# OliBus801/TARL-simulator

Hardware: AMD Instinct MI355X
Metric: ppo_env_steps_per_sec (higher is better)
Workload: dtype f32; 1 GPU; mpnn+ppo train, 10000-edge torus dual graph, 16384 agents, T=256 (BASELINE config 4); envs_per_gpu=32768, parallelism=dp1, rollout_kernels=frames

## Files before the change

### tarl-simulator_amd/csrc/critic.hip

```cpp
#include "tarl_common.h"

#define CR_H 64
#define CR_BM 128
#define CR_BK 32
#define CR_THREADS 256

typedef float f32x16 __attribute__((ext_vector_type(16)));

struct CriticParams {
  const float* w1;
  const float* b1;
  const float* w2;
  const float* b2;
  const float* w3;
  const float* b3;
};

__device__ __forceinline__ int mfma_row(int reg, int lane) { return (reg & 3) + 8 * (reg >> 2) + 4 * (lane >> 5); }

template <typename XT>
__global__ __launch_bounds__(CR_THREADS) void k_critic_fwd(const XT* __restrict__ counts, int64_t ldc, int64_t rps,
                                                           int64_t M, int64_t N,
                                                           const float* __restrict__ time_rows,
                                                           int64_t rows_per_time, CriticParams P,
                                                           float* __restrict__ value, float* __restrict__ h1_out,
                                                           float* __restrict__ h2_out) {
  __shared__ float lds[CR_H * (CR_BM + 1) + CR_H * (CR_H + 1)];
  float* Xs = lds;
  float* Ws = lds + CR_BK * (CR_BM + 1);
  const int tid = threadIdx.x, lane = tid & 63, wave = tid >> 6;
  const int64_t row0 = (int64_t)blockIdx.x * CR_BM;
  const int64_t ldw = N + 1;

  f32x16 acc0 = {0}, acc1 = {0};
  for (int64_t k0 = 0; k0 < N; k0 += CR_BK) {
    if (rps == 0) {
#pragma unroll
      for (int it = 0; it < (CR_BM * CR_BK) / CR_THREADS; ++it) {
        const int idx = it * CR_THREADS + tid;
        const int r = idx >> 5, k = idx & 31;
        const int64_t gr = row0 + r, gk = k0 + k;
        Xs[k * (CR_BM + 1) + r] = (gr < M && gk < N) ? (float)counts[gr * ldc + gk] : 0.0f;
      }
    } else {
      const int64_t slab_base = (row0 / rps) * (N * rps) + (row0 % rps);
#pragma unroll
      for (int it = 0; it < (CR_BM * CR_BK) / CR_THREADS; ++it) {
        const int idx = it * CR_THREADS + tid;
        const int r = idx & (CR_BM - 1), k = idx >> 7;
        const int64_t gr = row0 + r, gk = k0 + k;
        Xs[k * (CR_BM + 1) + r] = (gr < M && gk < N) ? (float)counts[slab_base + gk * rps + r] : 0.0f;
      }
    }
#pragma unroll
    for (int it = 0; it < (CR_H * CR_BK) / CR_THREADS; ++it) {
      const int idx = it * CR_THREADS + tid;
      const int j = idx >> 5, k = idx & 31;
      const int64_t gk = k0 + k;
      Ws[k * (CR_H + 1) + j] = (gk < N) ? P.w1[(int64_t)j * ldw + gk] : 0.0f;
    }
    __syncthreads();
#pragma unroll
    for (int kk = 0; kk < CR_BK; kk += 2) {
      const int k = kk + (lane >> 5);
      const float a = Xs[k * (CR_BM + 1) + wave * 32 + (lane & 31)];
      const float b0 = Ws[k * (CR_H + 1) + (lane & 31)];
      const float b1 = Ws[k * (CR_H + 1) + 32 + (lane & 31)];
      acc0 = __builtin_amdgcn_mfma_f32_32x32x2f32(a, b0, acc0, 0, 0, 0);
      acc1 = __builtin_amdgcn_mfma_f32_32x32x2f32(a, b1, acc1, 0, 0, 0);
    }
    __syncthreads();
  }

  float* Hs = lds;
  float* W2s = lds + CR_H * (CR_BM + 1);
  {
    const int j0 = lane & 31;
    const float wt0 = P.w1[(int64_t)j0 * ldw + N], wt1 = P.w1[(int64_t)(j0 + 32) * ldw + N];
    const float bb0 = P.b1[j0], bb1 = P.b1[j0 + 32];
#pragma unroll
    for (int r = 0; r < 16; ++r) {
      const int lr = wave * 32 + mfma_row(r, lane);
      const int64_t gr = row0 + lr;
      const float tm = (gr < M) ? time_rows[gr / rows_per_time] : 0.0f;
      float v0 = acc0[r] + tm * wt0 + bb0;
      float v1 = acc1[r] + tm * wt1 + bb1;
      v0 = v0 > 0.0f ? v0 : 0.0f;
      v1 = v1 > 0.0f ? v1 : 0.0f;
      Hs[j0 * (CR_BM + 1) + lr] = v0;
      Hs[(j0 + 32) * (CR_BM + 1) + lr] = v1;
      if (h1_out && gr < M) {
        h1_out[gr * CR_H + j0] = v0;
        h1_out[gr * CR_H + j0 + 32] = v1;
      }
    }
  }
#pragma unroll
  for (int it = 0; it < (CR_H * CR_H) / CR_THREADS; ++it) {
    const int idx = it * CR_THREADS + tid;
    const int j = idx >> 6, k = idx & 63;
    W2s[k * (CR_H + 1) + j] = P.w2[j * CR_H + k];
  }
  __syncthreads();
  f32x16 c0 = {0}, c1 = {0};
#pragma unroll
  for (int kk = 0; kk < CR_H; kk += 2) {
    const int k = kk + (lane >> 5);
    const float a = Hs[k * (CR_BM + 1) + wave * 32 + (lane & 31)];
    const float b0 = W2s[k * (CR_H + 1) + (lane & 31)];
    const float b1 = W2s[k * (CR_H + 1) + 32 + (lane & 31)];
    c0 = __builtin_amdgcn_mfma_f32_32x32x2f32(a, b0, c0, 0, 0, 0);
    c1 = __builtin_amdgcn_mfma_f32_32x32x2f32(a, b1, c1, 0, 0, 0);
  }
  __syncthreads();
  {
    const int j0 = lane & 31;
    const float bb0 = P.b2[j0], bb1 = P.b2[j0 + 32];
#pragma unroll
    for (int r = 0; r < 16; ++r) {
      const int lr = wave * 32 + mfma_row(r, lane);
      const int64_t gr = row0 + lr;
      float v0 = c0[r] + bb0, v1 = c1[r] + bb1;
      v0 = v0 > 0.0f ? v0 : 0.0f;
      v1 = v1 > 0.0f ? v1 : 0.0f;
      Hs[j0 * (CR_BM + 1) + lr] = v0;
      Hs[(j0 + 32) * (CR_BM + 1) + lr] = v1;
      if (h2_out && gr < M) {
        h2_out[gr * CR_H + j0] = v0;
        h2_out[gr * CR_H + j0 + 32] = v1;
      }
    }
  }
  __syncthreads();
  if (tid < CR_BM) {
    const int64_t gr = row0 + tid;
    if (gr < M) {
      float s = 0.0f;
#pragma unroll 8
      for (int j = 0; j < CR_H; ++j) s += Hs[j * (CR_BM + 1) + tid] * P.w3[j];
      value[gr] = s + P.b3[0];
    }
  }
}

#define CRS_LDX (CR_BM + 4)
__device__ __forceinline__ float4 load_x4(const float* p) { return *reinterpret_cast<const float4*>(p); }
__device__ __forceinline__ float4 load_x4(const uint8_t* p) {
  const uint32_t w = *reinterpret_cast<const uint32_t*>(p);
  return make_float4((float)(w & 255u), (float)((w >> 8) & 255u), (float)((w >> 16) & 255u), (float)(w >> 24));
}
template <typename XT>
__global__ __launch_bounds__(CR_THREADS) void k_critic_fwd_slab(const XT* __restrict__ counts, int64_t rps, int64_t M,
                                                                int64_t N, const float* __restrict__ time_rows,
                                                                int64_t rows_per_time, CriticParams P,
                                                                float* __restrict__ value) {
  __shared__ __attribute__((aligned(16))) float lds[2 * (CR_BK * CRS_LDX + CR_BK * (CR_H + 1))];
  const int XS = CR_BK * CRS_LDX, BUF = XS + CR_BK * (CR_H + 1);
  const int tid = threadIdx.x, lane = tid & 63, wave = tid >> 6;
  const int64_t row0 = (int64_t)blockIdx.x * CR_BM;
  const int64_t ldw = N + 1;
  const XT* xbase = counts + (row0 / rps) * (N * rps) + (row0 % rps);

  float4 xr[4];
  float wr[8];
  auto fetch = [&](int64_t k0) {
#pragma unroll
    for (int it = 0; it < 4; ++it) {
      const int idx = it * CR_THREADS + tid;
      const int r4 = (idx & 31) * 4, k = idx >> 5;
      const int64_t gk = k0 + k;
      xr[it] = (gk < N) ? load_x4(xbase + gk * rps + r4) : make_float4(0.f, 0.f, 0.f, 0.f);
    }
#pragma unroll
    for (int it = 0; it < 8; ++it) {
      const int idx = it * CR_THREADS + tid;
      const int j = idx >> 5, k = idx & 31;
      const int64_t gk = k0 + k;
      wr[it] = (gk < N) ? P.w1[(int64_t)j * ldw + gk] : 0.0f;
    }
  };
  auto stash = [&](int buf) {
    float* Xs = lds + buf * BUF;
    float* Ws = Xs + XS;
#pragma unroll
    for (int it = 0; it < 4; ++it) {
      const int idx = it * CR_THREADS + tid;
      const int r4 = (idx & 31) * 4, k = idx >> 5;
      *reinterpret_cast<float4*>(Xs + k * CRS_LDX + r4) = xr[it];
    }
#pragma unroll
    for (int it = 0; it < 8; ++it) {
      const int idx = it * CR_THREADS + tid;
      const int j = idx >> 5, k = idx & 31;
      Ws[k * (CR_H + 1) + j] = wr[it];
    }
  };

  f32x16 acc0 = {0}, acc1 = {0};
  fetch(0);
  stash(0);
  __syncthreads();
  int buf = 0;
  for (int64_t k0 = 0; k0 < N; k0 += CR_BK) {
    const bool more = k0 + CR_BK < N;
    if (more) fetch(k0 + CR_BK);
    const float* Xs = lds + buf * BUF;
    const float* Ws = Xs + XS;
#pragma unroll
    for (int kk = 0; kk < CR_BK; kk += 2) {
      const int k = kk + (lane >> 5);
      const float a = Xs[k * CRS_LDX + wave * 32 + (lane & 31)];
      const float b0 = Ws[k * (CR_H + 1) + (lane & 31)];
      const float b1 = Ws[k * (CR_H + 1) + 32 + (lane & 31)];
      acc0 = __builtin_amdgcn_mfma_f32_32x32x2f32(a, b0, acc0, 0, 0, 0);
      acc1 = __builtin_amdgcn_mfma_f32_32x32x2f32(a, b1, acc1, 0, 0, 0);
    }
    if (more) stash(buf ^ 1);
    __syncthreads();
    buf ^= 1;
  }

  float* Hs = lds;
  float* W2s = lds + CR_H * (CR_BM + 1);
  {
    const int j0 = lane & 31;
    const float wt0 = P.w1[(int64_t)j0 * ldw + N], wt1 = P.w1[(int64_t)(j0 + 32) * ldw + N];
    const float bb0 = P.b1[j0], bb1 = P.b1[j0 + 32];
#pragma unroll
    for (int r = 0; r < 16; ++r) {
      const int lr = wave * 32 + mfma_row(r, lane);
      const int64_t gr = row0 + lr;
      const float tm = (gr < M) ? time_rows[gr / rows_per_time] : 0.0f;
      float v0 = acc0[r] + tm * wt0 + bb0;
      float v1 = acc1[r] + tm * wt1 + bb1;
      v0 = v0 > 0.0f ? v0 : 0.0f;
      v1 = v1 > 0.0f ? v1 : 0.0f;
      Hs[j0 * (CR_BM + 1) + lr] = v0;
      Hs[(j0 + 32) * (CR_BM + 1) + lr] = v1;
    }
  }
#pragma unroll
  for (int it = 0; it < (CR_H * CR_H) / CR_THREADS; ++it) {
    const int idx = it * CR_THREADS + tid;
    const int j = idx >> 6, k = idx & 63;
    W2s[k * (CR_H + 1) + j] = P.w2[j * CR_H + k];
  }
  __syncthreads();
  f32x16 c0 = {0}, c1 = {0};
#pragma unroll
  for (int kk = 0; kk < CR_H; kk += 2) {
    const int k = kk + (lane >> 5);
    const float a = Hs[k * (CR_BM + 1) + wave * 32 + (lane & 31)];
    const float b0 = W2s[k * (CR_H + 1) + (lane & 31)];
    const float b1 = W2s[k * (CR_H + 1) + 32 + (lane & 31)];
    c0 = __builtin_amdgcn_mfma_f32_32x32x2f32(a, b0, c0, 0, 0, 0);
    c1 = __builtin_amdgcn_mfma_f32_32x32x2f32(a, b1, c1, 0, 0, 0);
  }
  __syncthreads();
  {
    const int j0 = lane & 31;
    const float bb0 = P.b2[j0], bb1 = P.b2[j0 + 32];
#pragma unroll
    for (int r = 0; r < 16; ++r) {
      const int lr = wave * 32 + mfma_row(r, lane);
      float v0 = c0[r] + bb0, v1 = c1[r] + bb1;
      v0 = v0 > 0.0f ? v0 : 0.0f;
      v1 = v1 > 0.0f ? v1 : 0.0f;
      Hs[j0 * (CR_BM + 1) + lr] = v0;
      Hs[(j0 + 32) * (CR_BM + 1) + lr] = v1;
    }
  }
  __syncthreads();
  if (tid < CR_BM) {
    const int64_t gr = row0 + tid;
    if (gr < M) {
      float s = 0.0f;
#pragma unroll 8
      for (int j = 0; j < CR_H; ++j) s += Hs[j * (CR_BM + 1) + tid] * P.w3[j];
      value[gr] = s + P.b3[0];
    }
  }
}

typedef __bf16 cbf16x8 __attribute__((ext_vector_type(8)));
#define CB_XLD 36
#define CB_WLD 40

__device__ __forceinline__ uint16_t cr_bf16_rne(float f) {
  uint32_t u = __float_as_uint(f);
  u += 0x7fffu + ((u >> 16) & 1u);
  return (uint16_t)(u >> 16);
}

__global__ __launch_bounds__(CR_THREADS) void k_split_w1(const float* __restrict__ w1, int64_t N, int64_t Kpad,
                                                         uint16_t* __restrict__ w3) {
  const int64_t idx = (int64_t)blockIdx.x * CR_THREADS + threadIdx.x;
  if (idx >= CR_H * Kpad) return;
  const int64_t j = idx / Kpad, k = idx - j * Kpad;
  const float w = k < N ? w1[j * (N + 1) + k] : 0.0f;
  const uint16_t hi = cr_bf16_rne(w);
  const float r1 = w - __uint_as_float((uint32_t)hi << 16);
  const uint16_t mid = cr_bf16_rne(r1);
  const float r2 = r1 - __uint_as_float((uint32_t)mid << 16);
  const uint16_t lo = cr_bf16_rne(r2);
  w3[idx] = hi;
  w3[CR_H * Kpad + idx] = mid;
  w3[2 * CR_H * Kpad + idx] = lo;
}

template <int CT>
__global__ __launch_bounds__(CR_THREADS) void k_critic_fwd_slab_u8x3(const uint8_t* __restrict__ counts, int64_t rps,
                                                                     int64_t M, int64_t N, int64_t Kpad,
                                                                     const float* __restrict__ time_rows,
                                                                     int64_t rows_per_time,
                                                                     const uint16_t* __restrict__ w3, CriticParams P,
                                                                     float* __restrict__ value) {
  constexpr int XB = CT * CR_BM * CB_XLD, WB = 3 * CR_H * CB_WLD * 2, BUF = XB + WB;
  constexpr int EPI = (CR_H * (CR_BM + 1) + CR_H * (CR_H + 1)) * 4;
  __shared__ __attribute__((aligned(16))) uint8_t lds_raw[2 * BUF > EPI ? 2 * BUF : EPI];
  static_assert(CR_BK == 32 && CR_BM == 128 && CR_THREADS == 256 && (CR_BM * CB_XLD) % 16 == 0, "X staging plan");
  const int tid = threadIdx.x, lane = tid & 63, wave = tid >> 6;
  const int64_t row0 = (int64_t)blockIdx.x * (CR_BM * CT);
  const int64_t ldw = N + 1;
  const uint8_t* xbase = counts + (row0 / rps) * (N * rps) + (row0 % rps);
  const int64_t WP = CR_H * Kpad;

  struct XStage {
    uint32_t xr[CT][4];
  };
  typedef uint32_t cu32x4 __attribute__((ext_vector_type(4)));
  struct WStage {
    cu32x4 p0, p1, p2;
  };
  const int64_t NIT = (N + CR_BK - 1) / CR_BK;
  const uint8_t* xthread = xbase + (int64_t)(4 * (tid >> 5)) * rps + 4 * (tid & 31);
  auto fetch_x = [&](XStage& st, int64_t it) __attribute__((always_inline)) {
    const int64_t k0 = (it < NIT ? it : NIT - 1) * CR_BK;
    if (k0 + CR_BK <= N) {
      const uint8_t* xk = xthread + k0 * rps;
#pragma unroll
      for (int i = 0; i < 4; ++i) {
#pragma unroll
        for (int c = 0; c < CT; ++c) st.xr[c][i] = *reinterpret_cast<const uint32_t*>(xk + CR_BM * c);
        xk += rps;
      }
    } else {
      const int kg = tid >> 5, eg = tid & 31;
#pragma unroll
      for (int i = 0; i < 4; ++i) {
        const int64_t k = k0 + 4 * kg + i;
        const uint8_t* xk = xbase + (k < N ? k : N - 1) * rps + 4 * eg;
#pragma unroll
        for (int c = 0; c < CT; ++c) st.xr[c][i] = *reinterpret_cast<const uint32_t*>(xk + CR_BM * c);
      }
    }
  };
  auto fetch_w = [&](WStage& st, int64_t it) __attribute__((always_inline)) {
    const int64_t k0 = (it < NIT ? it : NIT - 1) * CR_BK;
    const int j = tid >> 2, q = tid & 3;
    const uint16_t* wp = w3 + (int64_t)j * Kpad + k0 + 8 * q;
    st.p0 = *reinterpret_cast<const cu32x4*>(wp);
    st.p1 = *reinterpret_cast<const cu32x4*>(wp + WP);
    st.p2 = *reinterpret_cast<const cu32x4*>(wp + 2 * WP);
  };
  auto stash = [&](const XStage& sx, const WStage& sw, int buf) __attribute__((always_inline)) {
    uint8_t* Xs = lds_raw + buf * BUF;
    uint16_t* Wb = reinterpret_cast<uint16_t*>(Xs + XB);
    const int kg = tid >> 5, eg = tid & 31;
#pragma unroll
    for (int c = 0; c < CT; ++c) {
      const uint32_t r0 = sx.xr[c][0], r1 = sx.xr[c][1], r2 = sx.xr[c][2], r3 = sx.xr[c][3];
      const uint32_t a_lo = __builtin_amdgcn_perm(r1, r0, 0x05010400u), a_hi = __builtin_amdgcn_perm(r1, r0, 0x07030602u);
      const uint32_t b_lo = __builtin_amdgcn_perm(r3, r2, 0x05010400u), b_hi = __builtin_amdgcn_perm(r3, r2, 0x07030602u);
      const uint32_t v[4] = {__builtin_amdgcn_perm(b_lo, a_lo, 0x05040100u), __builtin_amdgcn_perm(b_lo, a_lo, 0x07060302u),
                             __builtin_amdgcn_perm(b_hi, a_hi, 0x05040100u), __builtin_amdgcn_perm(b_hi, a_hi, 0x07060302u)};
#pragma unroll
      for (int e = 0; e < 4; ++e) *reinterpret_cast<uint32_t*>(Xs + (CR_BM * c + 4 * eg + e) * CB_XLD + 4 * kg) = v[e];
    }
    const int j = tid >> 2, q = tid & 3;
    *reinterpret_cast<cu32x4*>(Wb + (0 * CR_H + j) * CB_WLD + 8 * q) = sw.p0;
    *reinterpret_cast<cu32x4*>(Wb + (1 * CR_H + j) * CB_WLD + 8 * q) = sw.p1;
    *reinterpret_cast<cu32x4*>(Wb + (2 * CR_H + j) * CB_WLD + 8 * q) = sw.p2;
  };

  f32x16 acc0[CT], acc1[CT];
#pragma unroll
  for (int c = 0; c < CT; ++c) {
    acc0[c] = (f32x16){0};
    acc1[c] = (f32x16){0};
  }
  const int r32 = lane & 31, h8 = (lane >> 5) * 8;
  auto multiply = [&](int buf) __attribute__((always_inline)) {
    const uint8_t* Xs = lds_raw + buf * BUF;
    const uint16_t* Wb = reinterpret_cast<const uint16_t*>(Xs + XB);
#pragma unroll
    for (int s = 0; s < CR_BK / 16; ++s) {
      cbf16x8 bx[CT];
#pragma unroll
      for (int c = 0; c < CT; ++c) {
        const uint32_t* xw = reinterpret_cast<const uint32_t*>(Xs + (CR_BM * c + wave * 32 + r32) * CB_XLD + 16 * s + h8);
        const uint32_t x0 = xw[0], x1 = xw[1];
        uint32_t bw[4];
#pragma unroll
        for (int j = 0; j < 4; ++j) {
          const uint32_t xs = j < 2 ? x0 : x1;
          const float c0 = (float)((xs >> (16 * (j & 1))) & 0xFFu), c1 = (float)((xs >> (16 * (j & 1) + 8)) & 0xFFu);
          bw[j] = __builtin_amdgcn_perm(__float_as_uint(c1), __float_as_uint(c0), 0x07060302u);
        }
        bx[c] = __builtin_bit_cast(cbf16x8, bw);
      }
#pragma unroll
      for (int pc = 0; pc < 3; ++pc) {
        const cbf16x8 a0 = *reinterpret_cast<const cbf16x8*>(Wb + (pc * CR_H + r32) * CB_WLD + 16 * s + h8);
        const cbf16x8 a1 = *reinterpret_cast<const cbf16x8*>(Wb + (pc * CR_H + 32 + r32) * CB_WLD + 16 * s + h8);
#pragma unroll
        for (int c = 0; c < CT; ++c) {
          acc0[c] = __builtin_amdgcn_mfma_f32_32x32x16_bf16(a0, bx[c], acc0[c], 0, 0, 0);
          acc1[c] = __builtin_amdgcn_mfma_f32_32x32x16_bf16(a1, bx[c], acc1[c], 0, 0, 0);
        }
      }
    }
  };
  XStage x0, x1, x2, x3;
  WStage w0, w1;
  fetch_w(w0, 0);
  fetch_x(x0, 0);
  fetch_w(w1, 1);
  fetch_x(x1, 1);
  fetch_x(x2, 2);
  fetch_x(x3, 3);
  stash(x0, w0, 0);
  __syncthreads();
#define CR_STEP(T_, XA_, XB_, WA_, WB_, BUF_)                                           \
  {                                                                                     \
    fetch_w(WA_, (T_) + 2);                                                             \
    fetch_x(XA_, (T_) + 4);                                                             \
    if ((T_) < NIT) multiply(BUF_);           \
    stash(XB_, WB_, (BUF_) ^ 1);                                                        \
    __syncthreads();                                                                    \
  }
  for (int64_t it = 0; it < NIT; it += 4) {
    CR_STEP(it, x0, x1, w0, w1, 0);
    CR_STEP(it + 1, x1, x2, w1, w0, 1);
    CR_STEP(it + 2, x2, x3, w0, w1, 0);
    CR_STEP(it + 3, x3, x0, w1, w0, 1);
  }
#undef CR_STEP

  float* Hs = reinterpret_cast<float*>(lds_raw);
  float* W2s = Hs + CR_H * (CR_BM + 1);
#pragma unroll
  for (int it = 0; it < (CR_H * CR_H) / CR_THREADS; ++it) {
    const int idx = it * CR_THREADS + tid;
    const int j = idx >> 6, k = idx & 63;
    W2s[k * (CR_H + 1) + j] = P.w2[j * CR_H + k];
  }
#pragma unroll
  for (int c = 0; c < CT; ++c) {
    const int64_t rowc = row0 + CR_BM * c;
    {
      const int lr = wave * 32 + r32;
      const int64_t gr = rowc + lr;
      const float tm = (gr < M) ? time_rows[gr / rows_per_time] : 0.0f;
#pragma unroll
      for (int r = 0; r < 16; ++r) {
        const int j = mfma_row(r, lane);
        float v0 = acc0[c][r] + tm * P.w1[(int64_t)j * ldw + N] + P.b1[j];
        float v1 = acc1[c][r] + tm * P.w1[(int64_t)(j + 32) * ldw + N] + P.b1[j + 32];
        Hs[j * (CR_BM + 1) + lr] = v0 > 0.0f ? v0 : 0.0f;
        Hs[(j + 32) * (CR_BM + 1) + lr] = v1 > 0.0f ? v1 : 0.0f;
      }
    }
    __syncthreads();
    f32x16 c0 = {0}, c1 = {0};
#pragma unroll
    for (int kk = 0; kk < CR_H; kk += 2) {
      const int k = kk + (lane >> 5);
      const float a = Hs[k * (CR_BM + 1) + wave * 32 + (lane & 31)];
      const float b0 = W2s[k * (CR_H + 1) + (lane & 31)];
      const float b1 = W2s[k * (CR_H + 1) + 32 + (lane & 31)];
      c0 = __builtin_amdgcn_mfma_f32_32x32x2f32(a, b0, c0, 0, 0, 0);
      c1 = __builtin_amdgcn_mfma_f32_32x32x2f32(a, b1, c1, 0, 0, 0);
    }
    __syncthreads();
    {
      const int j0 = lane & 31;
      const float bb0 = P.b2[j0], bb1 = P.b2[j0 + 32];
#pragma unroll
      for (int r = 0; r < 16; ++r) {
        const int lr = wave * 32 + mfma_row(r, lane);
        float v0 = c0[r] + bb0, v1 = c1[r] + bb1;
        v0 = v0 > 0.0f ? v0 : 0.0f;
        v1 = v1 > 0.0f ? v1 : 0.0f;
        Hs[j0 * (CR_BM + 1) + lr] = v0;
        Hs[(j0 + 32) * (CR_BM + 1) + lr] = v1;
      }
    }
    __syncthreads();
    if (tid < CR_BM) {
      const int64_t gr = rowc + tid;
      if (gr < M) {
        float sacc = 0.0f;
#pragma unroll 8
        for (int j = 0; j < CR_H; ++j) sacc += Hs[j * (CR_BM + 1) + tid] * P.w3[j];
        value[gr] = sacc + P.b3[0];
      }
    }
    __syncthreads();
  }
}

__global__ __launch_bounds__(CR_H) void k_critic_bwd_rows(int64_t M, const float* __restrict__ dv,
                                                          const float* __restrict__ h1, const float* __restrict__ h2,
                                                          CriticParams P, float* __restrict__ dh1,
                                                          float* __restrict__ dh2) {
  __shared__ float s_dh2[CR_H];
  const int64_t m = blockIdx.x;
  const int j = threadIdx.x;
  const float g = dv[m];
  const float d2 = (h2[m * CR_H + j] > 0.0f) ? g * P.w3[j] : 0.0f;
  s_dh2[j] = d2;
  dh2[m * CR_H + j] = d2;
  __syncthreads();
  float s = 0.0f;
  for (int i = 0; i < CR_H; ++i) s += s_dh2[i] * P.w2[i * CR_H + j];
  dh1[m * CR_H + j] = (h1[m * CR_H + j] > 0.0f) ? s : 0.0f;
}

__global__ __launch_bounds__(CR_THREADS) void k_critic_bwd_small(int64_t M, const float* __restrict__ dv,
                                                                 const float* __restrict__ h1,
                                                                 const float* __restrict__ h2,
                                                                 const float* __restrict__ dh1,
                                                                 const float* __restrict__ dh2,
                                                                 const float* __restrict__ time_rows,
                                                                 int64_t rows_per_time, int64_t N,
                                                                 float* __restrict__ gw1, float* __restrict__ gb1,
                                                                 float* __restrict__ gw2, float* __restrict__ gb2,
                                                                 float* __restrict__ gw3, float* __restrict__ gb3) {
  const int idx = blockIdx.x * CR_THREADS + threadIdx.x;
  if (idx < CR_H * CR_H) {
    const int j = idx >> 6, k = idx & 63;
    float s = 0.0f;
    for (int64_t m = 0; m < M; ++m) s += dh2[m * CR_H + j] * h1[m * CR_H + k];
    gw2[idx] += s;
  }
  if (idx < CR_H) {
    float sb2 = 0.0f, sb1 = 0.0f, sw3 = 0.0f, swt = 0.0f;
    for (int64_t m = 0; m < M; ++m) {
      sb2 += dh2[m * CR_H + idx];
      sb1 += dh1[m * CR_H + idx];
      sw3 += dv[m] * h2[m * CR_H + idx];
      swt += dh1[m * CR_H + idx] * time_rows[m / rows_per_time];
    }
    gb2[idx] += sb2;
    gb1[idx] += sb1;
    gw3[idx] += sw3;
    gw1[(int64_t)idx * (N + 1) + N] += swt;
  }
  if (idx == 0) {
    float s = 0.0f;
    for (int64_t m = 0; m < M; ++m) s += dv[m];
    gb3[0] += s;
  }
}

__global__ __launch_bounds__(CR_THREADS) void k_critic_bwd_w1(int64_t M, int64_t N, const float* __restrict__ counts,
                                                              int64_t ldc, const float* __restrict__ dh1,
                                                              float* __restrict__ gw1) {
  const int64_t k = (int64_t)blockIdx.x * CR_THREADS + threadIdx.x;
  const int j = blockIdx.y;
  if (k >= N) return;
  float s = 0.0f;
  for (int64_t m = 0; m < M; ++m) s += dh1[m * CR_H + j] * counts[m * ldc + k];
  gw1[(int64_t)j * (N + 1) + k] += s;
}

#define CB_RC 128
#define CB_RS 32
#define CB_SMALL (CR_H * CR_H + 4 * CR_H + 1)

__global__ __launch_bounds__(CR_THREADS) void k_critic_bwd_w1_part(int64_t M, int64_t N, const float* __restrict__ counts,
                                                                   int64_t ldc, const float* __restrict__ dh1,
                                                                   float* __restrict__ part) {
  __shared__ float4 s_dh[CB_RC * (CR_H / 4)];
  const int tid = threadIdx.x;
  const int64_t m0 = (int64_t)blockIdx.y * CB_RC;
  const int rows = (int)((M - m0) < CB_RC ? (M - m0) : CB_RC);
  const float4* src = reinterpret_cast<const float4*>(dh1 + m0 * CR_H);
  for (int e = tid; e < rows * (CR_H / 4); e += CR_THREADS) s_dh[e] = src[e];
  __syncthreads();
  const int kk = tid & 63, jg = tid >> 6;
  const int64_t k = (int64_t)blockIdx.x * 64 + kk;
  float acc[16];
#pragma unroll
  for (int i = 0; i < 16; ++i) acc[i] = 0.0f;
  if (k < N) {
    const float* col = counts + m0 * ldc + k;
#pragma unroll 4
    for (int m = 0; m < rows; ++m) {
      const float x = col[(int64_t)m * ldc];
#pragma unroll
      for (int q = 0; q < 4; ++q) {
        const float4 d = s_dh[m * (CR_H / 4) + jg * 4 + q];
        acc[4 * q + 0] = fmaf(d.x, x, acc[4 * q + 0]);
        acc[4 * q + 1] = fmaf(d.y, x, acc[4 * q + 1]);
        acc[4 * q + 2] = fmaf(d.z, x, acc[4 * q + 2]);
        acc[4 * q + 3] = fmaf(d.w, x, acc[4 * q + 3]);
      }
    }
    float* out = part + ((int64_t)blockIdx.y * CR_H + jg * 16) * N + k;
#pragma unroll
    for (int i = 0; i < 16; ++i) out[(int64_t)i * N] = acc[i];
  }
}

__global__ __launch_bounds__(CR_THREADS) void k_critic_bwd_w1_reduce(int64_t S, int64_t N, const float* __restrict__ part,
                                                                     float* __restrict__ gw1) {
  const int64_t idx = (int64_t)blockIdx.x * CR_THREADS + threadIdx.x;
  if (idx >= CR_H * N) return;
  const int64_t j = idx / N, k = idx - j * N;
  float s = 0.0f;
  for (int64_t c = 0; c < S; ++c) s += part[c * CR_H * N + idx];
  gw1[j * (N + 1) + k] += s;
}

__global__ __launch_bounds__(CR_THREADS) void k_critic_bwd_small_part(int64_t M, const float* __restrict__ dv,
                                                                      const float* __restrict__ h1,
                                                                      const float* __restrict__ h2,
                                                                      const float* __restrict__ dh1,
                                                                      const float* __restrict__ dh2,
                                                                      const float* __restrict__ time_rows,
                                                                      int64_t rows_per_time, float* __restrict__ part) {
  __shared__ float s_dh2[CB_RS * CR_H], s_h1[CB_RS * CR_H], s_dh1[CB_RS * CR_H], s_h2[CB_RS * CR_H];
  __shared__ float s_dv[CB_RS], s_tm[CB_RS];
  const int tid = threadIdx.x;
  const int64_t m0 = (int64_t)blockIdx.x * CB_RS;
  const int rows = (int)((M - m0) < CB_RS ? (M - m0) : CB_RS);
  for (int e = tid; e < CB_RS * CR_H; e += CR_THREADS) {
    const bool in = e < rows * CR_H;
    s_dh2[e] = in ? dh2[m0 * CR_H + e] : 0.0f;
    s_h1[e] = in ? h1[m0 * CR_H + e] : 0.0f;
    s_dh1[e] = in ? dh1[m0 * CR_H + e] : 0.0f;
    s_h2[e] = in ? h2[m0 * CR_H + e] : 0.0f;
  }
  if (tid < CB_RS) {
    s_dv[tid] = tid < rows ? dv[m0 + tid] : 0.0f;
    s_tm[tid] = tid < rows ? time_rows[(m0 + tid) / rows_per_time] : 0.0f;
  }
  __syncthreads();
  float* out = part + (int64_t)blockIdx.x * CB_SMALL;
  {
    const int j = tid >> 2, k0 = (tid & 3) * 16;
    float acc[16];
#pragma unroll
    for (int i = 0; i < 16; ++i) acc[i] = 0.0f;
    for (int m = 0; m < CB_RS; ++m) {
      const float a = s_dh2[m * CR_H + j];
#pragma unroll
      for (int i = 0; i < 16; ++i) acc[i] = fmaf(a, s_h1[m * CR_H + k0 + i], acc[i]);
    }
#pragma unroll
    for (int i = 0; i < 16; ++i) out[j * CR_H + k0 + i] = acc[i];
  }
  if (tid < CR_H) {
    float sb2 = 0.0f, sb1 = 0.0f, sw3 = 0.0f, swt = 0.0f;
    for (int m = 0; m < CB_RS; ++m) {
      sb2 += s_dh2[m * CR_H + tid];
      sb1 += s_dh1[m * CR_H + tid];
      sw3 = fmaf(s_dv[m], s_h2[m * CR_H + tid], sw3);
      swt = fmaf(s_dh1[m * CR_H + tid], s_tm[m], swt);
    }
    out[CR_H * CR_H + tid] = sb2;
    out[CR_H * CR_H + CR_H + tid] = sb1;
    out[CR_H * CR_H + 2 * CR_H + tid] = sw3;
    out[CR_H * CR_H + 3 * CR_H + tid] = swt;
  }
  if (tid == 0) {
    float sd = 0.0f;
    for (int m = 0; m < CB_RS; ++m) sd += s_dv[m];
    out[CB_SMALL - 1] = sd;
  }
}

__global__ __launch_bounds__(CR_THREADS) void k_critic_bwd_small_reduce(int64_t S, int64_t N, const float* __restrict__ part,
                                                                        float* __restrict__ gw1, float* __restrict__ gb1,
                                                                        float* __restrict__ gw2, float* __restrict__ gb2,
                                                                        float* __restrict__ gw3, float* __restrict__ gb3) {
  const int idx = blockIdx.x * CR_THREADS + threadIdx.x;
  if (idx >= CB_SMALL) return;
  float s = 0.0f;
  for (int64_t c = 0; c < S; ++c) s += part[c * CB_SMALL + idx];
  const int v = idx - CR_H * CR_H;
  if (v < 0)
    gw2[idx] += s;
  else if (v < CR_H)
    gb2[v] += s;
  else if (v < 2 * CR_H)
    gb1[v - CR_H] += s;
  else if (v < 3 * CR_H)
    gw3[v - 2 * CR_H] += s;
  else if (v < 4 * CR_H)
    gw1[(int64_t)(v - 3 * CR_H) * (N + 1) + N] += s;
  else
    gb3[0] += s;
}

#define CB_MANY_ROWS 512

template <typename XT>
static int critic_fwd(const XT* counts, int64_t ldc, int64_t rps, int64_t M, int64_t N, const float* time_rows,
                      int64_t rows_per_time, const float* w1, const float* b1, const float* w2, const float* b2,
                      const float* w3, const float* b3, float* value, float* h1_out, float* h2_out,
                      tarl_stream stream) {
  TARL_REQUIRE(counts && time_rows && w1 && b1 && w2 && b2 && w3 && b3 && value, "null argument");
  TARL_REQUIRE(M >= 1 && N >= 1 && rows_per_time >= 1, "bad sizes");
  TARL_REQUIRE(ceil_div(M, CR_BM) < ((int64_t)1 << 31), "too many rows");
  const CriticParams P{w1, b1, w2, b2, w3, b3};
  hipLaunchKernelGGL(k_critic_fwd<XT>, dim3((unsigned)ceil_div(M, CR_BM)), dim3(CR_THREADS), 0, (hipStream_t)stream,
                     counts, ldc, rps, M, N, time_rows, rows_per_time, P, value, h1_out, h2_out);
  TARL_LAUNCH_CHECK();
  return TARL_OK;
}

extern "C" int tarl_critic_mlp_fwd(const float* counts, int64_t ldc, int64_t M, int64_t N, const float* time_rows,
                                   int64_t rows_per_time, const float* w1, const float* b1, const float* w2,
                                   const float* b2, const float* w3, const float* b3, float* value, float* h1_out,
                                   float* h2_out, tarl_stream stream) {
  TARL_REQUIRE(ldc >= N, "row stride smaller than N");
  return critic_fwd(counts, ldc, 0, M, N, time_rows, rows_per_time, w1, b1, w2, b2, w3, b3, value, h1_out, h2_out,
                    stream);
}

extern "C" int tarl_critic_mlp_fwd_u8(const uint8_t* counts, int64_t ldc, int64_t M, int64_t N, const float* time_rows,
                                      int64_t rows_per_time, const float* w1, const float* b1, const float* w2,
                                      const float* b2, const float* w3, const float* b3, float* value, float* h1_out,
                                      float* h2_out, tarl_stream stream) {
  TARL_REQUIRE(ldc >= N, "row stride smaller than N");
  return critic_fwd(counts, ldc, 0, M, N, time_rows, rows_per_time, w1, b1, w2, b2, w3, b3, value, h1_out, h2_out,
                    stream);
}

#define CK_KC 64
#define CK_RB 32

__global__ __launch_bounds__(CR_THREADS) void k_critic_splitk_partial(const float* __restrict__ counts, int64_t ldc,
                                                                      int64_t M, int64_t N,
                                                                      const float* __restrict__ w1,
                                                                      float* __restrict__ partial, int64_t Mpad) {
  __shared__ float Xs[CK_RB * (CK_KC + 1)];
  __shared__ float Ws[CK_KC * (CR_H + 1)];
  const int tid = threadIdx.x;
  const int64_t k0 = (int64_t)blockIdx.x * CK_KC, row0 = (int64_t)blockIdx.y * CK_RB, ldw = N + 1;
#pragma unroll
  for (int it = 0; it < (CK_RB * CK_KC) / CR_THREADS; ++it) {
    const int idx = it * CR_THREADS + tid;
    const int r = idx >> 6, k = idx & 63;
    const int64_t gr = row0 + r, gk = k0 + k;
    Xs[r * (CK_KC + 1) + k] = (gr < M && gk < N) ? counts[gr * ldc + gk] : 0.0f;
  }
#pragma unroll
  for (int it = 0; it < (CR_H * CK_KC) / CR_THREADS; ++it) {
    const int idx = it * CR_THREADS + tid;
    const int j = idx >> 6, k = idx & 63;
    const int64_t gk = k0 + k;
    Ws[k * (CR_H + 1) + j] = (gk < N) ? w1[(int64_t)j * ldw + gk] : 0.0f;
  }
  __syncthreads();
  const int r = tid >> 3, jg = tid & 7;
  float acc[8] = {0, 0, 0, 0, 0, 0, 0, 0};
#pragma unroll 8
  for (int k = 0; k < CK_KC; ++k) {
    const float x = Xs[r * (CK_KC + 1) + k];
#pragma unroll
    for (int i = 0; i < 8; ++i) acc[i] = fmaf(x, Ws[k * (CR_H + 1) + jg + 8 * i], acc[i]);
  }
  float* out = partial + ((int64_t)blockIdx.x * Mpad + row0 + r) * CR_H;
#pragma unroll
  for (int i = 0; i < 8; ++i) out[jg + 8 * i] = acc[i];
}

__global__ __launch_bounds__(CR_THREADS) void k_critic_splitk_finish(const float* __restrict__ partial, int64_t S,
                                                                     int64_t Mpad, int64_t M, int64_t N,
                                                                     const float* __restrict__ time_rows,
                                                                     int64_t rows_per_time, CriticParams P,
                                                                     float* __restrict__ value,
                                                                     float* __restrict__ h1_out,
                                                                     float* __restrict__ h2_out) {
  __shared__ float H1[CK_RB * (CR_H + 1)];
  __shared__ float H2[CK_RB * (CR_H + 1)];
  __shared__ float W2s[CR_H * (CR_H + 1)];
  const int tid = threadIdx.x;
  const int64_t row0 = (int64_t)blockIdx.x * CK_RB, ldw = N + 1;
#pragma unroll
  for (int it = 0; it < (CR_H * CR_H) / CR_THREADS; ++it) {
    const int idx = it * CR_THREADS + tid;
    const int j = idx >> 6, k = idx & 63;
    W2s[k * (CR_H + 1) + j] = P.w2[j * CR_H + k];
  }
  const int r = tid >> 3, jg = tid & 7;
  const int64_t gr = row0 + r;
  const float tm = (gr < M) ? time_rows[gr / rows_per_time] : 0.0f;
  {
    float acc[8] = {0, 0, 0, 0, 0, 0, 0, 0};
    for (int64_t s = 0; s < S; ++s) {
      const float* in = partial + (s * Mpad + gr) * CR_H;
#pragma unroll
      for (int i = 0; i < 8; ++i) acc[i] += in[jg + 8 * i];
    }
#pragma unroll
    for (int i = 0; i < 8; ++i) {
      const int j = jg + 8 * i;
      float v = acc[i] + tm * P.w1[(int64_t)j * ldw + N] + P.b1[j];
      v = v > 0.0f ? v : 0.0f;
      H1[r * (CR_H + 1) + j] = v;
      if (h1_out && gr < M) h1_out[gr * CR_H + j] = v;
    }
  }
  __syncthreads();
  {
    float acc[8] = {0, 0, 0, 0, 0, 0, 0, 0};
#pragma unroll 8
    for (int k = 0; k < CR_H; ++k) {
      const float x = H1[r * (CR_H + 1) + k];
#pragma unroll
      for (int i = 0; i < 8; ++i) acc[i] = fmaf(x, W2s[k * (CR_H + 1) + jg + 8 * i], acc[i]);
    }
#pragma unroll
    for (int i = 0; i < 8; ++i) {
      const int j = jg + 8 * i;
      float v = acc[i] + P.b2[j];
      v = v > 0.0f ? v : 0.0f;
      H2[r * (CR_H + 1) + j] = v;
      if (h2_out && gr < M) h2_out[gr * CR_H + j] = v;
    }
  }
  __syncthreads();
  if (tid < CK_RB && row0 + tid < M) {
    float s = 0.0f;
#pragma unroll 8
    for (int j = 0; j < CR_H; ++j) s += H2[tid * (CR_H + 1) + j] * P.w3[j];
    value[row0 + tid] = s + P.b3[0];
  }
}

extern "C" int64_t tarl_critic_splitk_scratch_floats(int64_t M, int64_t N) {
  if (M < 1 || N < 1) return -1;
  return ceil_div(N, CK_KC) * ceil_div(M, CK_RB) * CK_RB * CR_H;
}

extern "C" int tarl_critic_mlp_fwd_splitk(const float* counts, int64_t ldc, int64_t M, int64_t N,
                                          const float* time_rows, int64_t rows_per_time, const float* w1,
                                          const float* b1, const float* w2, const float* b2, const float* w3,
                                          const float* b3, float* scratch, float* value, float* h1_out, float* h2_out,
                                          tarl_stream stream) {
  TARL_REQUIRE(counts && time_rows && w1 && b1 && w2 && b2 && w3 && b3 && value && scratch, "null argument");
  TARL_REQUIRE(M >= 1 && N >= 1 && rows_per_time >= 1 && ldc >= N, "bad sizes");
  const int64_t S = ceil_div(N, CK_KC), RB = ceil_div(M, CK_RB);
  TARL_REQUIRE(S < ((int64_t)1 << 31) && RB < 65536, "split-K critic: too many rows (use tarl_critic_mlp_fwd)");
  const CriticParams P{w1, b1, w2, b2, w3, b3};
  hipLaunchKernelGGL(k_critic_splitk_partial, dim3((unsigned)S, (unsigned)RB), dim3(CR_THREADS), 0, (hipStream_t)stream,
                     counts, ldc, M, N, w1, scratch, RB * CK_RB);
  TARL_LAUNCH_CHECK();
  hipLaunchKernelGGL(k_critic_splitk_finish, dim3((unsigned)RB), dim3(CR_THREADS), 0, (hipStream_t)stream, scratch, S,
                     RB * CK_RB, M, N, time_rows, rows_per_time, P, value, h1_out, h2_out);
  TARL_LAUNCH_CHECK();
  return TARL_OK;
}

template <typename XT>
static int critic_fwd_slabs(const XT* counts, int64_t rows_per_slab, int64_t M, int64_t N, const float* time_rows,
                            int64_t rows_per_time, const float* w1, const float* b1, const float* w2, const float* b2,
                            const float* w3, const float* b3, float* value, tarl_stream stream) {
  TARL_REQUIRE(rows_per_slab >= CR_BM && rows_per_slab % CR_BM == 0, "rows_per_slab must be a multiple of 128");
  TARL_REQUIRE(M % rows_per_slab == 0, "M must be a whole number of slabs");
  TARL_REQUIRE(counts && time_rows && w1 && b1 && w2 && b2 && w3 && b3 && value, "null argument");
  TARL_REQUIRE(M >= 1 && N >= 1 && rows_per_time >= 1, "bad sizes");
  TARL_REQUIRE(((uintptr_t)counts) % 16 == 0, "counts must be 16-byte aligned");
  const CriticParams P{w1, b1, w2, b2, w3, b3};
  hipLaunchKernelGGL(k_critic_fwd_slab<XT>, dim3((unsigned)(M / CR_BM)), dim3(CR_THREADS), 0, (hipStream_t)stream, counts,
                     rows_per_slab, M, N, time_rows, rows_per_time, P, value);
  TARL_LAUNCH_CHECK();
  return TARL_OK;
}

extern "C" int tarl_critic_mlp_fwd_slabs(const float* counts, int64_t rows_per_slab, int64_t M, int64_t N,
                                         const float* time_rows, int64_t rows_per_time, const float* w1,
                                         const float* b1, const float* w2, const float* b2, const float* w3,
                                         const float* b3, float* value, tarl_stream stream) {
  return critic_fwd_slabs(counts, rows_per_slab, M, N, time_rows, rows_per_time, w1, b1, w2, b2, w3, b3, value, stream);
}

extern "C" int64_t tarl_critic_split_scratch_bytes(int64_t N) {
  return N >= 1 ? 3 * CR_H * ceil_div(N, CR_BK) * CR_BK * (int64_t)sizeof(uint16_t) : -1;
}

extern "C" int tarl_critic_mlp_fwd_slabs_u8(const uint8_t* counts, int64_t rows_per_slab, int64_t M, int64_t N,
                                            const float* time_rows, int64_t rows_per_time, const float* w1,
                                            const float* b1, const float* w2, const float* b2, const float* w3,
                                            const float* b3, void* split_scratch, float* value, tarl_stream stream) {
  if (!split_scratch)
    return critic_fwd_slabs(counts, rows_per_slab, M, N, time_rows, rows_per_time, w1, b1, w2, b2, w3, b3, value, stream);
  TARL_REQUIRE(rows_per_slab >= CR_BM && rows_per_slab % CR_BM == 0, "rows_per_slab must be a multiple of 128");
  TARL_REQUIRE(M % rows_per_slab == 0, "M must be a whole number of slabs");
  TARL_REQUIRE(counts && time_rows && w1 && b1 && w2 && b2 && w3 && b3 && value, "null argument");
  TARL_REQUIRE(M >= 1 && N >= 1 && rows_per_time >= 1, "bad sizes");
  TARL_REQUIRE(((uintptr_t)counts) % 16 == 0 && ((uintptr_t)split_scratch) % 16 == 0, "counts / scratch must be 16-byte aligned");
  const int64_t Kpad = ceil_div(N, CR_BK) * CR_BK;
  const CriticParams P{w1, b1, w2, b2, w3, b3};
  hipStream_t s = (hipStream_t)stream;
  hipLaunchKernelGGL(k_split_w1, dim3((unsigned)ceil_div(CR_H * Kpad, CR_THREADS)), dim3(CR_THREADS), 0, s, w1, N, Kpad,
                     (uint16_t*)split_scratch);
  TARL_LAUNCH_CHECK();
  const char* ct_knob = getenv("TARL_CRITIC_CT");
  const int ct_env = ct_knob ? atoi(ct_knob) : 0;
  int ct = 1;
  if (rows_per_slab % (2 * CR_BM) == 0 && M / (2 * CR_BM) >= 1024) ct = 2;
  if ((ct_env == 1 || ct_env == 2 || ct_env == 4) && rows_per_slab % (ct_env * CR_BM) == 0) ct = ct_env;
  const dim3 grid((unsigned)(M / (CR_BM * ct)));
  if (ct == 4)
    hipLaunchKernelGGL(k_critic_fwd_slab_u8x3<4>, grid, dim3(CR_THREADS), 0, s, counts, rows_per_slab, M, N, Kpad, time_rows,
                       rows_per_time, (const uint16_t*)split_scratch, P, value);
  else if (ct == 2)
    hipLaunchKernelGGL(k_critic_fwd_slab_u8x3<2>, grid, dim3(CR_THREADS), 0, s, counts, rows_per_slab, M, N, Kpad, time_rows,
                       rows_per_time, (const uint16_t*)split_scratch, P, value);
  else
    hipLaunchKernelGGL(k_critic_fwd_slab_u8x3<1>, grid, dim3(CR_THREADS), 0, s, counts, rows_per_slab, M, N, Kpad, time_rows,
                       rows_per_time, (const uint16_t*)split_scratch, P, value);
  TARL_LAUNCH_CHECK();
  return TARL_OK;
}

extern "C" int64_t tarl_critic_mlp_bwd_scratch_floats(int64_t M, int64_t N) {
  if (M < 1 || N < 1) return -1;
  int64_t n = 2 * M * CR_H;
  if (M >= CB_MANY_ROWS) n += ceil_div(M, CB_RC) * CR_H * N + ceil_div(M, CB_RS) * CB_SMALL;
  return n;
}

extern "C" int tarl_critic_mlp_bwd(const float* counts, int64_t ldc, int64_t M, int64_t N, const float* time_rows,
                                   int64_t rows_per_time, const float* w1, const float* w2, const float* w3,
                                   const float* h1, const float* h2, const float* grad_value, float* scratch,
                                   float* gw1, float* gb1, float* gw2, float* gb2, float* gw3, float* gb3,
                                   tarl_stream stream) {
  TARL_REQUIRE(counts && time_rows && w1 && w2 && w3 && h1 && h2 && grad_value && scratch, "null argument");
  TARL_REQUIRE(gw1 && gb1 && gw2 && gb2 && gw3 && gb3, "null gradient buffer");
  TARL_REQUIRE(M >= 1 && N >= 1 && ldc >= N && rows_per_time >= 1, "bad sizes");
  TARL_REQUIRE(M < ((int64_t)1 << 31), "too many rows");
  const CriticParams P{w1, nullptr, w2, nullptr, w3, nullptr};
  float* dh1 = scratch;
  float* dh2 = scratch + M * CR_H;
  hipStream_t s = (hipStream_t)stream;
  hipLaunchKernelGGL(k_critic_bwd_rows, dim3((unsigned)M), dim3(CR_H), 0, s, M, grad_value, h1, h2, P, dh1, dh2);
  TARL_LAUNCH_CHECK();
  if (M >= CB_MANY_ROWS) {
    const int64_t S1 = ceil_div(M, CB_RC), S2 = ceil_div(M, CB_RS);
    TARL_REQUIRE(S1 < 65536, "too many rows for one launch");
    float* part_w1 = scratch + 2 * M * CR_H;
    float* part_small = part_w1 + S1 * CR_H * N;
    hipLaunchKernelGGL(k_critic_bwd_w1_part, dim3((unsigned)ceil_div(N, 64), (unsigned)S1), dim3(CR_THREADS), 0, s, M, N, counts,
                       ldc, dh1, part_w1);
    TARL_LAUNCH_CHECK();
    hipLaunchKernelGGL(k_critic_bwd_w1_reduce, dim3((unsigned)ceil_div(CR_H * N, CR_THREADS)), dim3(CR_THREADS), 0, s, S1, N,
                       part_w1, gw1);
    TARL_LAUNCH_CHECK();
    hipLaunchKernelGGL(k_critic_bwd_small_part, dim3((unsigned)S2), dim3(CR_THREADS), 0, s, M, grad_value, h1, h2, dh1, dh2,
                       time_rows, rows_per_time, part_small);
    TARL_LAUNCH_CHECK();
    hipLaunchKernelGGL(k_critic_bwd_small_reduce, dim3((unsigned)ceil_div(CB_SMALL, CR_THREADS)), dim3(CR_THREADS), 0, s, S2, N,
                       part_small, gw1, gb1, gw2, gb2, gw3, gb3);
    TARL_LAUNCH_CHECK();
    return TARL_OK;
  }
  hipLaunchKernelGGL(k_critic_bwd_small, dim3((CR_H * CR_H) / CR_THREADS), dim3(CR_THREADS), 0, s, M, grad_value, h1, h2,
                     dh1, dh2, time_rows, rows_per_time, N, gw1, gb1, gw2, gb2, gw3, gb3);
  TARL_LAUNCH_CHECK();
  hipLaunchKernelGGL(k_critic_bwd_w1, dim3((unsigned)ceil_div(N, CR_THREADS), CR_H), dim3(CR_THREADS), 0, s, M, N,
                     counts, ldc, dh1, gw1);
  TARL_LAUNCH_CHECK();
  return TARL_OK;
}
```

Before: 44.65 million env-steps/s.

## Stage critic forward tiles via global_load_lds DMA ring instead of registers

```diff
diff --git a/tarl-simulator_amd/csrc/critic.hip b/tarl-simulator_amd/csrc/critic.hip
--- a/tarl-simulator_amd/csrc/critic.hip
+++ b/tarl-simulator_amd/csrc/critic.hip
@@ -1,4 +1,5 @@
 #include "tarl_common.h"
+#include <string.h>
 
 #define CR_H 64
 #define CR_BM 128
@@ -308,6 +309,12 @@
   w3[2 * CR_H * Kpad + idx] = lo;
 }
 
+#define CR_U8X3_EPI ((CR_H * (CR_BM + 1) + CR_H * (CR_H + 1)) * 4)
+template <int CT>
+__device__ __forceinline__ void critic_u8x3_tail(uint8_t* lds_raw, const f32x16 (&acc0)[CT], const f32x16 (&acc1)[CT],
+                                                 int64_t row0, int64_t M, int64_t N, const float* __restrict__ time_rows,
+                                                 int64_t rows_per_time, const CriticParams& P, float* __restrict__ value);
+
 template <int CT>
 __global__ __launch_bounds__(CR_THREADS) void k_critic_fwd_slab_u8x3(const uint8_t* __restrict__ counts, int64_t rps,
                                                                      int64_t M, int64_t N, int64_t Kpad,
@@ -316,12 +323,11 @@
                                                                      const uint16_t* __restrict__ w3, CriticParams P,
                                                                      float* __restrict__ value) {
   constexpr int XB = CT * CR_BM * CB_XLD, WB = 3 * CR_H * CB_WLD * 2, BUF = XB + WB;
-  constexpr int EPI = (CR_H * (CR_BM + 1) + CR_H * (CR_H + 1)) * 4;
+  constexpr int EPI = CR_U8X3_EPI;
   __shared__ __attribute__((aligned(16))) uint8_t lds_raw[2 * BUF > EPI ? 2 * BUF : EPI];
   static_assert(CR_BK == 32 && CR_BM == 128 && CR_THREADS == 256 && (CR_BM * CB_XLD) % 16 == 0, "X staging plan");
   const int tid = threadIdx.x, lane = tid & 63, wave = tid >> 6;
   const int64_t row0 = (int64_t)blockIdx.x * (CR_BM * CT);
-  const int64_t ldw = N + 1;
   const uint8_t* xbase = counts + (row0 / rps) * (N * rps) + (row0 % rps);
   const int64_t WP = CR_H * Kpad;
 
@@ -446,7 +452,15 @@
     CR_STEP(it + 3, x3, x0, w1, w0, 1);
   }
 #undef CR_STEP
-
+  critic_u8x3_tail<CT>(lds_raw, acc0, acc1, row0, M, N, time_rows, rows_per_time, P, value);
+}
+
+template <int CT>
+__device__ __forceinline__ void critic_u8x3_tail(uint8_t* lds_raw, const f32x16 (&acc0)[CT], const f32x16 (&acc1)[CT],
+                                                 int64_t row0, int64_t M, int64_t N, const float* __restrict__ time_rows,
+                                                 int64_t rows_per_time, const CriticParams& P, float* __restrict__ value) {
+  const int tid = threadIdx.x, lane = tid & 63, wave = tid >> 6, r32 = lane & 31;
+  const int64_t ldw = N + 1;
   float* Hs = reinterpret_cast<float*>(lds_raw);
   float* W2s = Hs + CR_H * (CR_BM + 1);
 #pragma unroll
@@ -508,6 +522,117 @@
     }
     __syncthreads();
   }
+}
+
+typedef __attribute__((address_space(3))) void cr_lds_void;
+typedef __attribute__((address_space(1))) const void cr_global_void;
+#define CR_DMA16(SRC_, DST_) __builtin_amdgcn_global_load_lds((cr_global_void*)(SRC_), (cr_lds_void*)(DST_), 16, 0, 0)
+#define CR_WAIT_VM(N_) asm volatile("s_waitcnt vmcnt(%0)" ::"n"(N_) : "memory")
+
+template <int CT, int WPC>
+__global__ __launch_bounds__(CR_THREADS, WPC) void k_critic_fwd_slab_u8x3_dma(const uint8_t* __restrict__ counts, int64_t rps,
+                                                                              int64_t M, int64_t N, int64_t Kpad,
+                                                                              const float* __restrict__ time_rows,
+                                                                              int64_t rows_per_time,
+                                                                              const uint16_t* __restrict__ w3, CriticParams P,
+                                                                              float* __restrict__ value) {
+  constexpr int XB = CT * CR_BM * CR_BK, WPB = CR_H * CR_BK * 2, WB = 3 * WPB, RING = 3 * XB + 2 * WB;
+  static_assert(CR_BK == 32 && CR_BM == 128 && CR_THREADS == 256 && CR_H == 64, "DMA plan");
+  static_assert(WPC * (RING > CR_U8X3_EPI ? RING : CR_U8X3_EPI) <= 160 * 1024, "LDS plan");
+  __shared__ __attribute__((aligned(16))) uint8_t lds_raw[RING > CR_U8X3_EPI ? RING : CR_U8X3_EPI];
+  const int tid = threadIdx.x, lane = tid & 63, wave = __builtin_amdgcn_readfirstlane(tid >> 6);
+  const int64_t row0 = (int64_t)blockIdx.x * (CR_BM * CT);
+  const uint8_t* xbase = counts + (row0 / rps) * (N * rps) + (row0 % rps);
+  const int64_t WP = CR_H * Kpad;
+  const int64_t NIT = (N + CR_BK - 1) / CR_BK;
+  int xrow[CT];
+  const uint8_t* xcol[CT];
+#pragma unroll
+  for (int i = 0; i < CT; ++i) {
+    const int idx = 64 * (CT * wave + i) + lane;
+    xrow[i] = idx / (8 * CT);
+    xcol[i] = xbase + 16 * (idx % (8 * CT));
+  }
+  const int wj = 16 * wave + (lane >> 2), wq = (lane & 3) ^ ((wj >> 2) & 3);
+  const uint16_t* wsrc = w3 + (int64_t)wj * Kpad + 8 * wq;
+  auto request_w = [&](int64_t it, int slot) __attribute__((always_inline)) {
+    const int64_t k0 = (it < NIT ? it : NIT - 1) * CR_BK;
+    uint8_t* dst = lds_raw + 3 * XB + slot * WB + 1024 * wave;
+#pragma unroll
+    for (int i = 0; i < 3; ++i) CR_DMA16(wsrc + i * WP + k0, dst + i * WPB);
+  };
+  auto request_x = [&](int64_t it, int slot) __attribute__((always_inline)) {
+    const int64_t k0 = (it < NIT ? it : NIT - 1) * CR_BK;
+    uint8_t* dst = lds_raw + slot * XB + 1024 * CT * wave;
+#pragma unroll
+    for (int i = 0; i < CT; ++i) {
+      const int64_t k = k0 + xrow[i];
+      CR_DMA16(xcol[i] + (k < N ? k : N - 1) * rps, dst + 1024 * i);
+    }
+  };
+  f32x16 acc0[CT], acc1[CT];
+#pragma unroll
+  for (int c = 0; c < CT; ++c) {
+    acc0[c] = (f32x16){0};
+    acc1[c] = (f32x16){0};
+  }
+  const int r32 = lane & 31, h = lane >> 5;
+  const int xoff = 8 * h * (CR_BM * CT) + 32 * (tid >> 6) + r32;
+  const int wsw = h ^ ((r32 >> 2) & 3);
+  const int woff[2] = {3 * XB + 16 * (4 * r32 + wsw), 3 * XB + 16 * (4 * r32 + (wsw ^ 2))};
+  auto load_b = [&](int slot, int s, cbf16x8 (&bx)[CT]) __attribute__((always_inline)) {
+    const uint8_t* Xs = lds_raw + slot * XB + xoff;
+#pragma unroll
+    for (int c = 0; c < CT; ++c) {
+      uint32_t bw[4];
+#pragma unroll
+      for (int j = 0; j < 4; ++j) {
+        const float c0 = (float)Xs[(16 * s + 2 * j) * (CR_BM * CT) + CR_BM * c];
+        const float c1 = (float)Xs[(16 * s + 2 * j + 1) * (CR_BM * CT) + CR_BM * c];
+        bw[j] = __builtin_amdgcn_perm(__float_as_uint(c1), __float_as_uint(c0), 0x07060302u);
+      }
+      bx[c] = __builtin_bit_cast(cbf16x8, bw);
+    }
+  };
+  auto mfma_step = [&](int slot, int s, const cbf16x8 (&bx)[CT]) __attribute__((always_inline)) {
+#pragma unroll
+    for (int pc = 0; pc < 3; ++pc) {
+      const uint8_t* Wb = lds_raw + slot * WB + woff[s] + pc * WPB;
+      const cbf16x8 a0 = *reinterpret_cast<const cbf16x8*>(Wb);
+      const cbf16x8 a1 = *reinterpret_cast<const cbf16x8*>(Wb + 32 * 64);
+#pragma unroll
+      for (int c = 0; c < CT; ++c) {
+        acc0[c] = __builtin_amdgcn_mfma_f32_32x32x16_bf16(a0, bx[c], acc0[c], 0, 0, 0);
+        acc1[c] = __builtin_amdgcn_mfma_f32_32x32x16_bf16(a1, bx[c], acc1[c], 0, 0, 0);
+      }
+    }
+  };
+  request_w(0, 0);
+  request_x(0, 0);
+  request_x(1, 1);
+  CR_WAIT_VM(0);
+  __builtin_amdgcn_s_barrier();
+  cbf16x8 b0[CT], b1[CT];
+  load_b(0, 0, b0);
+  int x0 = 0, x1 = 1, x2 = 2, w0 = 0;
+  for (int64_t t = 0; t < NIT; ++t) {
+    request_w(t + 1, w0 ^ 1);
+    request_x(t + 2, x2);
+    load_b(x0, 1, b1);
+    mfma_step(w0, 0, b0);
+    load_b(x1, 0, b0);
+    mfma_step(w0, 1, b1);
+    CR_WAIT_VM(0);
+    asm volatile("s_waitcnt lgkmcnt(0)" ::: "memory");
+    __builtin_amdgcn_s_barrier();
+    const int xt = x0;
+    x0 = x1;
+    x1 = x2;
+    x2 = xt;
+    w0 ^= 1;
+  }
+  __syncthreads();
+  critic_u8x3_tail<CT>(lds_raw, acc0, acc1, row0, M, N, time_rows, rows_per_time, P, value);
 }
 
 __global__ __launch_bounds__(CR_H) void k_critic_bwd_rows(int64_t M, const float* __restrict__ dv,
@@ -911,12 +1036,25 @@
   hipLaunchKernelGGL(k_split_w1, dim3((unsigned)ceil_div(CR_H * Kpad, CR_THREADS)), dim3(CR_THREADS), 0, s, w1, N, Kpad,
                      (uint16_t*)split_scratch);
   TARL_LAUNCH_CHECK();
+  const char* stage_knob = getenv("TARL_CRITIC_STAGE");
+  const bool reg_staged = stage_knob && !strcmp(stage_knob, "reg");
   const char* ct_knob = getenv("TARL_CRITIC_CT");
   const int ct_env = ct_knob ? atoi(ct_knob) : 0;
   int ct = 1;
   if (rows_per_slab % (2 * CR_BM) == 0 && M / (2 * CR_BM) >= 1024) ct = 2;
+  if (!reg_staged && rows_per_slab % (4 * CR_BM) == 0 && M / (4 * CR_BM) >= 4096) ct = 4;
   if ((ct_env == 1 || ct_env == 2 || ct_env == 4) && rows_per_slab % (ct_env * CR_BM) == 0) ct = ct_env;
   const dim3 grid((unsigned)(M / (CR_BM * ct)));
+  if (!reg_staged && ct > 1) {
+    if (ct == 4)
+      hipLaunchKernelGGL((k_critic_fwd_slab_u8x3_dma<4, 2>), grid, dim3(CR_THREADS), 0, s, counts, rows_per_slab, M, N, Kpad,
+                         time_rows, rows_per_time, (const uint16_t*)split_scratch, P, value);
+    else
+      hipLaunchKernelGGL((k_critic_fwd_slab_u8x3_dma<2, 3>), grid, dim3(CR_THREADS), 0, s, counts, rows_per_slab, M, N, Kpad,
+                         time_rows, rows_per_time, (const uint16_t*)split_scratch, P, value);
+    TARL_LAUNCH_CHECK();
+    return TARL_OK;
+  }
   if (ct == 4)
     hipLaunchKernelGGL(k_critic_fwd_slab_u8x3<4>, grid, dim3(CR_THREADS), 0, s, counts, rows_per_slab, M, N, Kpad, time_rows,
                        rows_per_time, (const uint16_t*)split_scratch, P, value);
```

Result: no change. 44.84 million env-steps/s, median of 3 (+0.4%).
